# fudan-zvg/4d-gaussian-splatting

Measured on AMD Instinct MI355X. Metric: train-step images/sec + forward Mpix/s, 300k 4D Gaussians @1352x1014, higher is better.
Workload: dtype f32; 1 GPU; [model stored in Morton order, as fdgs.harness.train keeps it] C3: 300000 4D Gaussians, 1352x1014, SH degree 3 + time degree 2 (M=48), rot_4d=True, 4 views/GPU/step, L1+SSIM loss (fused HIP), Adam, fused activations, explicit fwd/loss/bwd on two HIP streams; num_rendered=2059257, cameras=4 different rotated off-axis cameras per step (fdgs.synth.POSES rig0..rig3), tile_cull=True, visible=254370, global_batch=4, parallelism=frame-parallel dp1, mode=weak scaling, 4 views per GPU and step (the reference's DyNeRF batch per GPU)

## Files before the change

4d-gaussian-splatting_amd/csrc/ssim.hip:

```cpp
#include <cstdlib>
#include "fdgs_common.h"

namespace fdgs
{
#ifndef FDGS_SSIM_STY
#define FDGS_SSIM_STY 32
#endif
	constexpr int STX = 32, STY = FDGS_SSIM_STY;
	constexpr int SROWS = STY / 8;
	constexpr int SR = 5;
	constexpr int SW = STX + 2 * SR;
	constexpr int SHH = STY + 2 * SR;
	constexpr int SSTR = 46;
	constexpr int SSTR1 = 48;
	constexpr int HSTR = 38;
	constexpr int HSTR1B = 36;
	constexpr int STHREADS = 256;
	typedef float v2f __attribute__((ext_vector_type(2)));
	typedef float v4f __attribute__((ext_vector_type(4)));

	struct TileId { int tx, ty, c, index; bool valid; };
	__device__ __forceinline__ TileId ssim_tile_of(int gx, int gy, int C)
	{
		const int total = gx * gy * C, chunk = (total + 7) / 8;
		const int wg = (int)blockIdx.x, xcd = wg & 7, k = wg >> 3;
		TileId t;
		t.index = xcd * chunk + k;
		t.valid = k < chunk && t.index < total;
		const int i = t.valid ? t.index : 0;
		t.c = i / (gx * gy);
		const int r = i - t.c * (gx * gy);
		t.ty = r / gx; t.tx = r - t.ty * gx;
		return t;
	}
	static inline int ssim_grid(int gx, int gy, int C) { return ((gx * gy * C + 7) / 8) * 8; }

	__device__ constexpr float GW[11] = {
		0.0010283801f, 0.0075987582f, 0.0360007733f, 0.1093606874f, 0.2130055279f, 0.2660117149f,
		0.2130055279f, 0.1093606874f, 0.0360007733f, 0.0075987582f, 0.0010283801f };

	__global__ void __launch_bounds__(STHREADS) ssim_fwd_kernel(
		const float* __restrict__ img1, const float* __restrict__ img2, int C, int H, int W,
		float* __restrict__ dm_dmu1, float* __restrict__ dm_de11, float* __restrict__ dm_de12,
		float* __restrict__ partial_l1, float* __restrict__ partial_ssim)
	{
		constexpr int IN_BYTES = SHH * SSTR * 8, HM_BYTES = SHH * HSTR * 8;
		constexpr int SH_BYTES = IN_BYTES > HM_BYTES ? IN_BYTES : HM_BYTES;
		__shared__ __attribute__((aligned(16))) char s_raw[HM_BYTES + SH_BYTES];
		v2f (*h_m)[HSTR] = reinterpret_cast<v2f (*)[HSTR]>(s_raw);
		v2f (*s_in)[SSTR] = reinterpret_cast<v2f (*)[SSTR]>(s_raw + HM_BYTES);
		v2f (*h_s)[HSTR] = reinterpret_cast<v2f (*)[HSTR]>(s_raw + HM_BYTES);
		__shared__ float red[2][STHREADS / WAVE];

		const TileId tile = ssim_tile_of((W + STX - 1) / STX, (H + STY - 1) / STY, C);
		if (!tile.valid) return;
		const int c = tile.c;
		const int x0 = tile.tx * STX, y0 = tile.ty * STY;
		const int tid = threadIdx.x;
		const size_t plane = (size_t)c * H * W;

		float l1 = 0.f;
		{
			constexpr int RPT = STHREADS / SW, TRIPS = (SHH + RPT - 1) / RPT;
			const int lyb = tid / SW, hx = tid - lyb * SW;
			const int gxh = x0 + hx - SR;
			const bool col_in = tid < RPT * SW && (unsigned)gxh < (unsigned)W;
			const bool col_own = (unsigned)(hx - SR) < (unsigned)STX;
			v2f p[TRIPS];
#pragma unroll
			for (int t = 0; t < TRIPS; t++)
			{
				const int ly = lyb + t * RPT, gy = y0 + ly - SR;
				const bool in = col_in && ly < SHH && (unsigned)gy < (unsigned)H;
				const size_t o = in ? plane + (size_t)gy * W + gxh : plane;
				const float vx = img1[o], vy = img2[o];
				p[t] = in ? v2f{ vx + vy, vx - vy } : v2f{ 0.0f, 0.0f };
			}
#pragma unroll
			for (int t = 0; t < TRIPS; t++)
			{
				const int ly = lyb + t * RPT;
				if (tid < RPT * SW && ly < SHH) s_in[ly][hx] = p[t];
				const bool own = col_own && (unsigned)(ly - SR) < (unsigned)STY;
				l1 += own ? fabsf(p[t].y) : 0.0f;
			}
		}
		__syncthreads();

		constexpr int HR = (SHH * (STX / 4) + STHREADS - 1) / STHREADS;
		v2f as[HR][4];
#pragma unroll
		for (int r = 0; r < HR; r++)
		{
			const int task = tid + r * STHREADS;
			if (task < SHH * (STX / 4))
			{
				const int ly = task >> 3, cx = (task & 7) * 4;
				v2f p[16], sq[14];
				const v4f* src = reinterpret_cast<const v4f*>(&s_in[ly][cx]);
#pragma unroll
				for (int i = 0; i < 7; i++) { const v4f q = src[i]; p[2 * i] = v2f{ q.x, q.y }; p[2 * i + 1] = v2f{ q.z, q.w }; }
#pragma unroll
				for (int i = 0; i < 14; i++) sq[i] = p[i] * p[i];
				v2f am[4];
#pragma unroll
				for (int j = 0; j < 4; j++)
				{
					am[j] = GW[0] * p[j]; as[r][j] = GW[0] * sq[j];
#pragma unroll
					for (int k = 1; k < 11; k++) { am[j] += GW[k] * p[j + k]; as[r][j] += GW[k] * sq[j + k]; }
				}
				v4f* dm = reinterpret_cast<v4f*>(&h_m[ly][cx]);
				dm[0] = v4f{ am[0].x, am[0].y, am[1].x, am[1].y }; dm[1] = v4f{ am[2].x, am[2].y, am[3].x, am[3].y };
			}
			__builtin_amdgcn_sched_barrier(0);
		}
		__syncthreads();
#pragma unroll
		for (int r = 0; r < HR; r++)
		{
			const int task = tid + r * STHREADS;
			if (task < SHH * (STX / 4))
			{
				const int ly = task >> 3, cx = (task & 7) * 4;
				v4f* ds = reinterpret_cast<v4f*>(&h_s[ly][cx]);
				ds[0] = v4f{ as[r][0].x, as[r][0].y, as[r][1].x, as[r][1].y }; ds[1] = v4f{ as[r][2].x, as[r][2].y, as[r][3].x, as[r][3].y };
			}
		}
		__syncthreads();

		const int lx = tid & (STX - 1), ly0 = (tid >> 5) * SROWS;
		v2f vm[10 + SROWS], vs[10 + SROWS];
#pragma unroll
		for (int r = 0; r < 10 + SROWS; r++) { vm[r] = h_m[ly0 + r][lx]; vs[r] = h_s[ly0 + r][lx]; }
		float sv = 0.f;
		const int gx = x0 + lx;
#pragma unroll
		for (int j = 0; j < SROWS; j++)
		{
			v2f mu = GW[0] * vm[j], e2 = GW[0] * vs[j];
#pragma unroll
			for (int k = 1; k < 11; k++) { mu += GW[k] * vm[j + k]; e2 += GW[k] * vs[j + k]; }
			const int gy = y0 + ly0 + j;
			if (gx < W && gy < H)
			{
				const float mu1 = 0.5f * (mu.x + mu.y), mu2 = 0.5f * (mu.x - mu.y);
				const float e_sum = 0.5f * (e2.x + e2.y), e12 = 0.25f * (e2.x - e2.y);
				const float C1 = 0.01f * 0.01f, C2 = 0.03f * 0.03f;
				const float mu1_sq = mu1 * mu1, mu2_sq = mu2 * mu2, mu12 = mu1 * mu2;
				const float sg12 = e12 - mu12;
				const float A = 2.f * mu12 + C1, B = 2.f * sg12 + C2, Cc = mu1_sq + mu2_sq + C1, D = (e_sum - (mu1_sq + mu2_sq)) + C2;
				const float rC = __builtin_amdgcn_rcpf(Cc), rD = __builtin_amdgcn_rcpf(D);
				const float inv = rC * rD;
				const float m = A * B * inv;
				const float dm_dA = B * inv, dm_dB = A * inv, dm_dC = -m * rC, dm_dD = -m * rD;
				const size_t o = plane + (size_t)gy * W + gx;
				dm_dmu1[o] = dm_dA * 2.f * mu2 - dm_dB * 2.f * mu2 + dm_dC * 2.f * mu1 - dm_dD * 2.f * mu1;
				dm_de11[o] = dm_dD;
				dm_de12[o] = 2.f * dm_dB;
				sv += m;
			}
		}
#pragma unroll
		for (int o = 32; o > 0; o >>= 1) { l1 += __shfl_down(l1, o); sv += __shfl_down(sv, o); }
		if ((tid & 63) == 0) { red[0][tid >> 6] = l1; red[1][tid >> 6] = sv; }
		__syncthreads();
		if (tid == 0)
		{
			const int b = tile.index;
			partial_l1[b] = red[0][0] + red[0][1] + red[0][2] + red[0][3];
			partial_ssim[b] = red[1][0] + red[1][1] + red[1][2] + red[1][3];
		}
	}

	__global__ void __launch_bounds__(STHREADS) ssim_bwd_kernel(
		const float* __restrict__ img1, const float* __restrict__ img2, int C, int H, int W,
		const float* __restrict__ dm_dmu1, const float* __restrict__ dm_de11, const float* __restrict__ dm_de12,
		const float* __restrict__ upstream, float w_l1, float w_ssim, float* __restrict__ dL_dimg1)
	{
		constexpr int SP_BYTES = SHH * SSTR * 8, SQ_BYTES = SHH * SSTR1 * 4, HP_BYTES = SHH * HSTR * 8, HQ_BYTES = SHH * HSTR1B * 4;
		constexpr int LDS_BYTES = SP_BYTES + SQ_BYTES > HP_BYTES + HQ_BYTES ? SP_BYTES + SQ_BYTES : HP_BYTES + HQ_BYTES;
		__shared__ __attribute__((aligned(16))) char s_raw[LDS_BYTES];
		v2f (*s_p)[SSTR] = reinterpret_cast<v2f (*)[SSTR]>(s_raw);
		float (*s_q)[SSTR1] = reinterpret_cast<float (*)[SSTR1]>(s_raw + SP_BYTES);
		v2f (*h_p)[HSTR] = reinterpret_cast<v2f (*)[HSTR]>(s_raw);
		float (*h_q)[HSTR1B] = reinterpret_cast<float (*)[HSTR1B]>(s_raw + HP_BYTES);

		const TileId tile = ssim_tile_of((W + STX - 1) / STX, (H + STY - 1) / STY, C);
		if (!tile.valid) return;
		const int c = tile.c;
		const int x0 = tile.tx * STX, y0 = tile.ty * STY;
		const int tid = threadIdx.x;
		const size_t plane = (size_t)c * H * W;

		{
			constexpr int RPT = STHREADS / SW, TRIPS = (SHH + RPT - 1) / RPT;
			const int lyb = tid / SW, hx = tid - lyb * SW;
			const int gxh = x0 + hx - SR;
			const bool col_in = tid < RPT * SW && (unsigned)gxh < (unsigned)W;
			v2f p[TRIPS];
			float q[TRIPS];
#pragma unroll
			for (int t = 0; t < TRIPS; t++)
			{
				const int ly = lyb + t * RPT, gy = y0 + ly - SR;
				const bool in = col_in && ly < SHH && (unsigned)gy < (unsigned)H;
				const size_t o = in ? plane + (size_t)gy * W + gxh : plane;
				const float va = dm_dmu1[o], vb = dm_de11[o], vc = dm_de12[o];
				p[t] = in ? v2f{ va, vb } : v2f{ 0.0f, 0.0f };
				q[t] = in ? vc : 0.0f;
			}
#pragma unroll
			for (int t = 0; t < TRIPS; t++)
			{
				const int ly = lyb + t * RPT;
				if (tid < RPT * SW && ly < SHH) { s_p[ly][hx] = p[t]; s_q[ly][hx] = q[t]; }
			}
		}
		const int lx = tid & (STX - 1), ly0 = (tid >> 5) * SROWS;
		const int gx = x0 + lx;
		float px[SROWS], py[SROWS];
#pragma unroll
		for (int j = 0; j < SROWS; j++)
		{
			const int gy = y0 + ly0 + j;
			const size_t o = (gx < W && gy < H) ? plane + (size_t)gy * W + gx : plane;
			px[j] = img1[o]; py[j] = img2[o];
		}
		__syncthreads();
		constexpr int HR = (SHH * (STX / 4) + STHREADS - 1) / STHREADS;
		v2f ap[HR][4];
		float aq[HR][4];
#pragma unroll
		for (int r = 0; r < HR; r++)
		{
			const int task = tid + r * STHREADS;
			if (task < SHH * (STX / 4))
			{
				const int ly = task >> 3, cx = (task & 7) * 4;
				v2f p[16];
				float q[16];
				const v4f* sp = reinterpret_cast<const v4f*>(&s_p[ly][cx]);
				const v4f* sq = reinterpret_cast<const v4f*>(&s_q[ly][cx]);
#pragma unroll
				for (int i = 0; i < 7; i++) { const v4f t = sp[i]; p[2 * i] = v2f{ t.x, t.y }; p[2 * i + 1] = v2f{ t.z, t.w }; }
#pragma unroll
				for (int i = 0; i < 4; i++) { const v4f t = sq[i]; q[4 * i] = t.x; q[4 * i + 1] = t.y; q[4 * i + 2] = t.z; q[4 * i + 3] = t.w; }
#pragma unroll
				for (int j = 0; j < 4; j++)
				{
					ap[r][j] = GW[0] * p[j]; aq[r][j] = GW[0] * q[j];
#pragma unroll
					for (int k = 1; k < 11; k++) { ap[r][j] += GW[k] * p[j + k]; aq[r][j] += GW[k] * q[j + k]; }
				}
			}
			__builtin_amdgcn_sched_barrier(0);
		}
		__syncthreads();
#pragma unroll
		for (int r = 0; r < HR; r++)
		{
			const int task = tid + r * STHREADS;
			if (task < SHH * (STX / 4))
			{
				const int ly = task >> 3, cx = (task & 7) * 4;
				v4f* dp = reinterpret_cast<v4f*>(&h_p[ly][cx]);
				dp[0] = v4f{ ap[r][0].x, ap[r][0].y, ap[r][1].x, ap[r][1].y }; dp[1] = v4f{ ap[r][2].x, ap[r][2].y, ap[r][3].x, ap[r][3].y };
				*reinterpret_cast<v4f*>(&h_q[ly][cx]) = v4f{ aq[r][0], aq[r][1], aq[r][2], aq[r][3] };
			}
		}
		__syncthreads();
		v2f vp[10 + SROWS];
		float vq[10 + SROWS];
#pragma unroll
		for (int r = 0; r < 10 + SROWS; r++) { vp[r] = h_p[ly0 + r][lx]; vq[r] = h_q[ly0 + r][lx]; }
		const float up = upstream[0];
#pragma unroll
		for (int j = 0; j < SROWS; j++)
		{
			v2f ab = GW[0] * vp[j];
			float d = GW[0] * vq[j];
#pragma unroll
			for (int k = 1; k < 11; k++) { ab += GW[k] * vp[j + k]; d += GW[k] * vq[j + k]; }
			const int gy = y0 + ly0 + j;
			if (gx < W && gy < H)
			{
				const size_t o = plane + (size_t)gy * W + gx;
				const float x = px[j], y = py[j];
				const float diff = x - y;
				const float sgn = diff > 0.f ? 1.f : (diff < 0.f ? -1.f : 0.f);
				dL_dimg1[o] = up * (w_l1 * sgn + w_ssim * (ab.x + 2.f * x * ab.y + y * d));
			}
		}
	}
}

namespace fdgs
{
	constexpr int FT = 32;
	constexpr int FB = FT + 2 * SR;
	constexpr int FA = FB + 2 * SR;
	constexpr int FBC = 44;
	constexpr int FSA = 54;
	constexpr int FSH = 46;
	constexpr int FSX = 48;
	constexpr int FSD = 46;
	constexpr int FSQ = 48;
	constexpr int FRV = 7;

	__device__ __forceinline__ void ssim_fused_body(
		const float* __restrict__ img1, const float* __restrict__ img2, int C, int H, int W,
		const float* __restrict__ upstream, float w_l1, float w_ssim, float* __restrict__ dL_dimg1,
		float* __restrict__ partial_l1, float* __restrict__ partial_ssim)
	{
		constexpr int R0_BYTES = FA * FSH * 8;
		constexpr int IN_BYTES = FA * FSA * 8, HS_BYTES = FA * FSH * 8, HX_BYTES = FA * FSX * 4;
		constexpr int R1_BYTES = IN_BYTES > HS_BYTES + HX_BYTES ? IN_BYTES : HS_BYTES + HX_BYTES;
		static_assert(FB * HSTR * 8 + FB * HSTR1B * 4 <= R0_BYTES, "h_p + h_q must fit where h_m was");
		static_assert(FB * FSD * 8 + FB * FSQ * 4 <= R1_BYTES, "d_p + d_q must fit where h_s + h_x were");
		__shared__ __attribute__((aligned(16))) char s_raw[R0_BYTES + R1_BYTES];
		v2f (*h_m)[FSH] = reinterpret_cast<v2f (*)[FSH]>(s_raw);
		v2f (*s_in)[FSA] = reinterpret_cast<v2f (*)[FSA]>(s_raw + R0_BYTES);
		v2f (*h_s)[FSH] = reinterpret_cast<v2f (*)[FSH]>(s_raw + R0_BYTES);
		float (*h_x)[FSX] = reinterpret_cast<float (*)[FSX]>(s_raw + R0_BYTES + HS_BYTES);
		v2f (*d_p)[FSD] = reinterpret_cast<v2f (*)[FSD]>(s_raw + R0_BYTES);
		float (*d_q)[FSQ] = reinterpret_cast<float (*)[FSQ]>(s_raw + R0_BYTES + FB * FSD * 8);
		v2f (*h_p)[HSTR] = reinterpret_cast<v2f (*)[HSTR]>(s_raw);
		float (*h_q)[HSTR1B] = reinterpret_cast<float (*)[HSTR1B]>(s_raw + FB * HSTR * 8);
		__shared__ float red[2][STHREADS / WAVE];

		const TileId tile = ssim_tile_of((W + FT - 1) / FT, (H + FT - 1) / FT, C);
		if (!tile.valid) return;
		const int c = tile.c;
		const int x0 = tile.tx * FT, y0 = tile.ty * FT;
		const int tid = threadIdx.x;
		const size_t plane = (size_t)c * H * W;

		float l1 = 0.f;
		{
			constexpr int RPT = STHREADS / FA, TRIPS = (FA + RPT - 1) / RPT;
			const int lyb = tid / FA, hx = tid - lyb * FA;
			const int gxh = x0 + hx - 2 * SR;
			const bool col_in = tid < RPT * FA && (unsigned)gxh < (unsigned)W;
			const bool col_own = (unsigned)(hx - 2 * SR) < (unsigned)FT;
			v2f p[TRIPS];
#pragma unroll
			for (int t = 0; t < TRIPS; t++)
			{
				const int ly = lyb + t * RPT, gy = y0 + ly - 2 * SR;
				const bool in = col_in && ly < FA && (unsigned)gy < (unsigned)H;
				const size_t o = in ? plane + (size_t)gy * W + gxh : plane;
				const float vx = img1[o], vy = img2[o];
				p[t] = in ? v2f{ vx, vy } : v2f{ 0.0f, 0.0f };
			}
#pragma unroll
			for (int t = 0; t < TRIPS; t++)
			{
				const int ly = lyb + t * RPT;
				if (tid < RPT * FA && ly < FA) s_in[ly][hx] = p[t];
				const bool own = col_own && (unsigned)(ly - 2 * SR) < (unsigned)FT;
				l1 += own ? fabsf(p[t].x - p[t].y) : 0.0f;
			}
			if (tid < FA) { s_in[tid][FA] = v2f{ 0.0f, 0.0f }; s_in[tid][FA + 1] = v2f{ 0.0f, 0.0f }; }
		}
		const int lx = tid & (FT - 1), ly0 = (tid >> 5) * SROWS;
		const int gx = x0 + lx;
		float px[SROWS], py[SROWS];
#pragma unroll
		for (int j = 0; j < SROWS; j++)
		{
			const int gy = y0 + ly0 + j;
			const size_t o = (gx < W && gy < H) ? plane + (size_t)gy * W + gx : plane;
			px[j] = img1[o]; py[j] = img2[o];
		}
		__syncthreads();

		{
			constexpr int GPR = FBC / 4, NT = FA * GPR, HR = (NT + STHREADS - 1) / STHREADS;
			v2f as[HR][4];
			float ax[HR][4];
#pragma unroll
			for (int r = 0; r < HR; r++)
			{
				const int task = tid + r * STHREADS;
				if (task < NT)
				{
					const int ly = task / GPR, cx = (task - ly * GPR) * 4;
					v2f p[16], sq[14];
					float xy[14];
					const v4f* src = reinterpret_cast<const v4f*>(&s_in[ly][cx]);
#pragma unroll
					for (int i = 0; i < 7; i++) { const v4f q = src[i]; p[2 * i] = v2f{ q.x, q.y }; p[2 * i + 1] = v2f{ q.z, q.w }; }
#pragma unroll
					for (int i = 0; i < 14; i++) { sq[i] = p[i] * p[i]; xy[i] = p[i].x * p[i].y; }
					v2f am[4];
#pragma unroll
					for (int j = 0; j < 4; j++)
					{
						am[j] = GW[0] * p[j]; as[r][j] = GW[0] * sq[j]; ax[r][j] = GW[0] * xy[j];
#pragma unroll
						for (int k = 1; k < 11; k++) { am[j] += GW[k] * p[j + k]; as[r][j] += GW[k] * sq[j + k]; ax[r][j] += GW[k] * xy[j + k]; }
					}
					v4f* dm = reinterpret_cast<v4f*>(&h_m[ly][cx]);
					dm[0] = v4f{ am[0].x, am[0].y, am[1].x, am[1].y }; dm[1] = v4f{ am[2].x, am[2].y, am[3].x, am[3].y };
				}
				__builtin_amdgcn_sched_barrier(0);
			}
			__syncthreads();
#pragma unroll
			for (int r = 0; r < HR; r++)
			{
				const int task = tid + r * STHREADS;
				if (task < NT)
				{
					const int ly = task / GPR, cx = (task - ly * GPR) * 4;
					v4f* ds = reinterpret_cast<v4f*>(&h_s[ly][cx]);
					ds[0] = v4f{ as[r][0].x, as[r][0].y, as[r][1].x, as[r][1].y }; ds[1] = v4f{ as[r][2].x, as[r][2].y, as[r][3].x, as[r][3].y };
					*reinterpret_cast<v4f*>(&h_x[ly][cx]) = v4f{ ax[r][0], ax[r][1], ax[r][2], ax[r][3] };
				}
			}
		}
		__syncthreads();

		float sv = 0.f;
		{
			const int bc = tid % FB, rg = tid / FB;
			const bool work = rg < FB / FRV;
			const int br0 = work ? rg * FRV : 0;
			v2f dp[FRV];
			float dq[FRV];
			{
				v2f vm[10 + FRV], vs[10 + FRV];
				float vx[10 + FRV];
#pragma unroll
				for (int r = 0; r < 10 + FRV; r++) { vm[r] = h_m[br0 + r][bc]; vs[r] = h_s[br0 + r][bc]; vx[r] = h_x[br0 + r][bc]; }
				const int gxb = x0 + bc - SR;
				const bool col_own = (unsigned)(bc - SR) < (unsigned)FT;
#pragma unroll
				for (int j = 0; j < FRV; j++)
				{
					v2f mu = GW[0] * vm[j], e2 = GW[0] * vs[j];
					float e12 = GW[0] * vx[j];
#pragma unroll
					for (int k = 1; k < 11; k++) { mu += GW[k] * vm[j + k]; e2 += GW[k] * vs[j + k]; e12 += GW[k] * vx[j + k]; }
					const int br = br0 + j, gyb = y0 + br - SR;
					dp[j] = v2f{ 0.0f, 0.0f }; dq[j] = 0.0f;
					if (work && (unsigned)gxb < (unsigned)W && (unsigned)gyb < (unsigned)H)
					{
						const float mu1 = mu.x, mu2 = mu.y, e11 = e2.x, e22 = e2.y;
						const float C1 = 0.01f * 0.01f, C2 = 0.03f * 0.03f;
						const float mu1_sq = mu1 * mu1, mu2_sq = mu2 * mu2, mu12 = mu1 * mu2;
						const float sg1 = e11 - mu1_sq, sg2 = e22 - mu2_sq, sg12 = e12 - mu12;
						const float A = 2.f * mu12 + C1, B = 2.f * sg12 + C2, Cc = mu1_sq + mu2_sq + C1, D = sg1 + sg2 + C2;
						const float rC = __builtin_amdgcn_rcpf(Cc), rD = __builtin_amdgcn_rcpf(D);
						const float inv = rC * rD;
						const float m = A * B * inv;
						const float dm_dA = B * inv, dm_dB = A * inv, dm_dC = -m * rC, dm_dD = -m * rD;
						dp[j] = v2f{ dm_dA * 2.f * mu2 - dm_dB * 2.f * mu2 + dm_dC * 2.f * mu1 - dm_dD * 2.f * mu1, dm_dD };
						dq[j] = 2.f * dm_dB;
						if (col_own && (unsigned)(br - SR) < (unsigned)FT) sv += m;
					}
				}
			}
			__syncthreads();
			if (work)
			{
#pragma unroll
				for (int j = 0; j < FRV; j++) { d_p[br0 + j][bc] = dp[j]; d_q[br0 + j][bc] = dq[j]; }
			}
			if (tid < FB) { d_q[tid][FB] = 0.0f; d_q[tid][FB + 1] = 0.0f; d_q[tid][FB + 2] = 0.0f; d_q[tid][FB + 3] = 0.0f; }
		}
		__syncthreads();

		{
			constexpr int NT = FB * (FT / 4), HR = (NT + STHREADS - 1) / STHREADS;
#pragma unroll
			for (int r = 0; r < HR; r++)
			{
				const int task = tid + r * STHREADS;
				if (task < NT)
				{
					const int ly = task >> 3, cx = (task & 7) * 4;
					v2f p[16];
					float q[16];
					const v4f* sp = reinterpret_cast<const v4f*>(&d_p[ly][cx]);
					const v4f* sq = reinterpret_cast<const v4f*>(&d_q[ly][cx]);
#pragma unroll
					for (int i = 0; i < 7; i++) { const v4f t = sp[i]; p[2 * i] = v2f{ t.x, t.y }; p[2 * i + 1] = v2f{ t.z, t.w }; }
#pragma unroll
					for (int i = 0; i < 4; i++) { const v4f t = sq[i]; q[4 * i] = t.x; q[4 * i + 1] = t.y; q[4 * i + 2] = t.z; q[4 * i + 3] = t.w; }
					v2f ap[4];
					float aq[4];
#pragma unroll
					for (int j = 0; j < 4; j++)
					{
						ap[j] = GW[0] * p[j]; aq[j] = GW[0] * q[j];
#pragma unroll
						for (int k = 1; k < 11; k++) { ap[j] += GW[k] * p[j + k]; aq[j] += GW[k] * q[j + k]; }
					}
					v4f* dpo = reinterpret_cast<v4f*>(&h_p[ly][cx]);
					dpo[0] = v4f{ ap[0].x, ap[0].y, ap[1].x, ap[1].y }; dpo[1] = v4f{ ap[2].x, ap[2].y, ap[3].x, ap[3].y };
					*reinterpret_cast<v4f*>(&h_q[ly][cx]) = v4f{ aq[0], aq[1], aq[2], aq[3] };
				}
				__builtin_amdgcn_sched_barrier(0);
			}
		}
		__syncthreads();

		{
			v2f vp[10 + SROWS];
			float vq[10 + SROWS];
#pragma unroll
			for (int r = 0; r < 10 + SROWS; r++) { vp[r] = h_p[ly0 + r][lx]; vq[r] = h_q[ly0 + r][lx]; }
			const float up = upstream[0];
#pragma unroll
			for (int j = 0; j < SROWS; j++)
			{
				v2f ab = GW[0] * vp[j];
				float d = GW[0] * vq[j];
#pragma unroll
				for (int k = 1; k < 11; k++) { ab += GW[k] * vp[j + k]; d += GW[k] * vq[j + k]; }
				const int gy = y0 + ly0 + j;
				if (gx < W && gy < H)
				{
					const size_t o = plane + (size_t)gy * W + gx;
					const float x = px[j], y = py[j];
					const float diff = x - y;
					const float sgn = diff > 0.f ? 1.f : (diff < 0.f ? -1.f : 0.f);
					dL_dimg1[o] = up * (w_l1 * sgn + w_ssim * (ab.x + 2.f * x * ab.y + y * d));
				}
			}
		}
#pragma unroll
		for (int o = 32; o > 0; o >>= 1) { l1 += __shfl_down(l1, o); sv += __shfl_down(sv, o); }
		if ((tid & 63) == 0) { red[0][tid >> 6] = l1; red[1][tid >> 6] = sv; }
		__syncthreads();
		if (tid == 0)
		{
			const int b = tile.index;
			partial_l1[b] = red[0][0] + red[0][1] + red[0][2] + red[0][3];
			partial_ssim[b] = red[1][0] + red[1][1] + red[1][2] + red[1][3];
		}
	}
}

namespace fdgs
{
#define FDGS_SSIM_FUSED_PARAMS const float* __restrict__ img1, const float* __restrict__ img2, int C, int H, int W, const float* __restrict__ upstream, \
		float w_l1, float w_ssim, float* __restrict__ dL_dimg1, float* __restrict__ partial_l1, float* __restrict__ partial_ssim
	__global__ void __launch_bounds__(STHREADS) __attribute__((amdgpu_waves_per_eu(3, 3))) ssim_fused_kernel(FDGS_SSIM_FUSED_PARAMS)
	{
		ssim_fused_body(img1, img2, C, H, W, upstream, w_l1, w_ssim, dL_dimg1, partial_l1, partial_ssim);
	}
	__global__ void __launch_bounds__(STHREADS) ssim_fused_kernel_wpe2(FDGS_SSIM_FUSED_PARAMS)
	{
		ssim_fused_body(img1, img2, C, H, W, upstream, w_l1, w_ssim, dL_dimg1, partial_l1, partial_ssim);
	}
#undef FDGS_SSIM_FUSED_PARAMS
}

extern "C" int fdgs_l1_ssim_value_and_grad(const float* img, const float* gt, int32_t C, int32_t H, int32_t W,
                                           const float* upstream, float lambda_dssim, float* dL_dimg,
                                           float* partial_l1, float* partial_ssim, void* stream)
{
	using namespace fdgs;
	static_assert(STY == 32 && SROWS == 4, "the fused kernel shares the 32-row tile's partial-sum layout with the two-kernel path");
	if (!img || !gt || !upstream || !dL_dimg || !partial_l1 || !partial_ssim || C <= 0 || H <= 0 || W <= 0) return FDGS_ERR_INVALID_ARG;
	const float n = (float)C * (float)H * (float)W;
	const float w_l1 = (1.0f - lambda_dssim) / n, w_ssim = -lambda_dssim / n;
	const dim3 grid(ssim_grid(div_up(W, FT), div_up(H, FT), C)), block(STHREADS, 1, 1);
	static const bool wpe2 = []() { const char* e = getenv("FDGS_SSIM_FUSED_WPE"); return e && e[0] == '2'; }();
	if (wpe2) hipLaunchKernelGGL(ssim_fused_kernel_wpe2, grid, block, 0, (hipStream_t)stream, img, gt, C, H, W, upstream, w_l1, w_ssim, dL_dimg, partial_l1, partial_ssim);
	else hipLaunchKernelGGL(ssim_fused_kernel, grid, block, 0, (hipStream_t)stream, img, gt, C, H, W, upstream, w_l1, w_ssim, dL_dimg, partial_l1, partial_ssim);
	return hipGetLastError() == hipSuccess ? FDGS_OK : FDGS_ERR_HIP;
}

extern "C" int fdgs_l1_ssim_forward(const float* img, const float* gt, int32_t C, int32_t H, int32_t W,
                                    float* dm_dmu1, float* dm_de11, float* dm_de12,
                                    float* partial_l1, float* partial_ssim, void* stream)
{
	using namespace fdgs;
	if (!img || !gt || !dm_dmu1 || !dm_de11 || !dm_de12 || !partial_l1 || !partial_ssim || C <= 0 || H <= 0 || W <= 0) return FDGS_ERR_INVALID_ARG;
	const dim3 grid(ssim_grid(div_up(W, STX), div_up(H, STY), C)), block(STHREADS, 1, 1);
	hipLaunchKernelGGL(ssim_fwd_kernel, grid, block, 0, (hipStream_t)stream, img, gt, C, H, W, dm_dmu1, dm_de11, dm_de12, partial_l1, partial_ssim);
	return hipGetLastError() == hipSuccess ? FDGS_OK : FDGS_ERR_HIP;
}

extern "C" int fdgs_l1_ssim_backward(const float* img, const float* gt, int32_t C, int32_t H, int32_t W,
                                     const float* dm_dmu1, const float* dm_de11, const float* dm_de12,
                                     const float* upstream, float lambda_dssim, float* dL_dimg, void* stream)
{
	using namespace fdgs;
	if (!img || !gt || !dm_dmu1 || !dm_de11 || !dm_de12 || !upstream || !dL_dimg || C <= 0 || H <= 0 || W <= 0) return FDGS_ERR_INVALID_ARG;
	const float n = (float)C * (float)H * (float)W;
	const float w_l1 = (1.0f - lambda_dssim) / n, w_ssim = -lambda_dssim / n;
	const dim3 grid(ssim_grid(div_up(W, STX), div_up(H, STY), C)), block(STHREADS, 1, 1);
	hipLaunchKernelGGL(ssim_bwd_kernel, grid, block, 0, (hipStream_t)stream, img, gt, C, H, W, dm_dmu1, dm_de11, dm_de12, upstream, w_l1, w_ssim, dL_dimg);
	return hipGetLastError() == hipSuccess ? FDGS_OK : FDGS_ERR_HIP;
}

namespace fdgs
{
	__global__ void __launch_bounds__(1024) l1_ssim_finish_kernel(const float* __restrict__ partial_l1, const float* __restrict__ partial_ssim,
	                                                              int nparts, float inv_n, float lambda_dssim, float* __restrict__ out, long long view_stride)
	{
		partial_l1 += (size_t)blockIdx.x * view_stride; partial_ssim += (size_t)blockIdx.x * view_stride; out += 3 * (size_t)blockIdx.x;
		__shared__ float r0[16], r1[16];
		float a = 0.f, b = 0.f;
		for (int base = 0; base < nparts; base += 8 * 1024)
		{
			float va[8], vb[8];
#pragma unroll
			for (int k = 0; k < 8; k++)
			{
				const int i = base + k * 1024 + (int)threadIdx.x;
				va[k] = i < nparts ? partial_l1[i] : 0.f;
				vb[k] = i < nparts ? partial_ssim[i] : 0.f;
			}
			a += ((va[0] + va[1]) + (va[2] + va[3])) + ((va[4] + va[5]) + (va[6] + va[7]));
			b += ((vb[0] + vb[1]) + (vb[2] + vb[3])) + ((vb[4] + vb[5]) + (vb[6] + vb[7]));
		}
#pragma unroll
		for (int o = 32; o > 0; o >>= 1) { a += __shfl_xor(a, o); b += __shfl_xor(b, o); }
		if ((threadIdx.x & 63) == 0) { r0[threadIdx.x >> 6] = a; r1[threadIdx.x >> 6] = b; }
		__syncthreads();
		if (threadIdx.x == 0)
		{
			float s0 = 0.f, s1 = 0.f;
			for (int w = 0; w < 16; w++) { s0 += r0[w]; s1 += r1[w]; }
			const float l1 = s0 * inv_n, ss = s1 * inv_n;
			out[0] = (1.0f - lambda_dssim) * l1 + lambda_dssim * (1.0f - ss);
			out[1] = l1;
			out[2] = ss;
		}
	}
}

extern "C" int fdgs_l1_ssim_loss(const float* partial_l1, const float* partial_ssim, int32_t num_partials, int32_t C, int32_t H, int32_t W,
                                 float lambda_dssim, float* loss_l1_ssim, void* stream)
{
	using namespace fdgs;
	if (!partial_l1 || !partial_ssim || !loss_l1_ssim || num_partials <= 0 || C <= 0 || H <= 0 || W <= 0) return FDGS_ERR_INVALID_ARG;
	const float inv_n = 1.0f / ((float)C * (float)H * (float)W);
	hipLaunchKernelGGL(l1_ssim_finish_kernel, dim3(1), dim3(1024), 0, (hipStream_t)stream, partial_l1, partial_ssim, num_partials, inv_n, lambda_dssim, loss_l1_ssim, 0ll);
	return hipGetLastError() == hipSuccess ? FDGS_OK : FDGS_ERR_HIP;
}

extern "C" int fdgs_l1_ssim_loss_batch(const float* partials, int32_t num_views, int32_t num_partials, int32_t C, int32_t H, int32_t W,
                                       float lambda_dssim, float* losses, void* stream)
{
	using namespace fdgs;
	if (!partials || !losses || num_views <= 0 || num_partials <= 0 || C <= 0 || H <= 0 || W <= 0) return FDGS_ERR_INVALID_ARG;
	const float inv_n = 1.0f / ((float)C * (float)H * (float)W);
	hipLaunchKernelGGL(l1_ssim_finish_kernel, dim3(num_views), dim3(1024), 0, (hipStream_t)stream, partials, partials + num_partials, num_partials, inv_n,
	                   lambda_dssim, losses, 2ll * num_partials);
	return hipGetLastError() == hipSuccess ? FDGS_OK : FDGS_ERR_HIP;
}

extern "C" int fdgs_l1_ssim_num_partials(int32_t C, int32_t H, int32_t W)
{
	using namespace fdgs;
	return div_up(W, STX) * div_up(H, STY) * C;
}
```

Measured before the change: 2435 images/s.

## Reorder SSIM separable blur to vertical-in-registers then horizontal-from-LDS with vector stores

Rewrites the standalone SSIM forward and backward kernels. Each thread now loads a 6-row column strip from global memory straight into registers and does the vertical 11-tap blur there, with a fast unguarded path for interior tiles. The horizontal blur then runs from a single LDS buffer, with each thread producing 4 adjacent pixels and writing them with 16-byte vector stores when rows are aligned. This removes the raw-input LDS staging, one intermediate LDS pass and two barriers, in exchange for more registers per thread and some overlap between row groups, which recompute a few rows.

```diff
diff --git a/4d-gaussian-splatting_amd/csrc/ssim.hip b/4d-gaussian-splatting_amd/csrc/ssim.hip
--- a/4d-gaussian-splatting_amd/csrc/ssim.hip
+++ b/4d-gaussian-splatting_amd/csrc/ssim.hip
@@ -39,17 +39,37 @@
 		0.0010283801f, 0.0075987582f, 0.0360007733f, 0.1093606874f, 0.2130055279f, 0.2660117149f,
 		0.2130055279f, 0.1093606874f, 0.0360007733f, 0.0075987582f, 0.0010283801f };
 
+	constexpr int VR = 6;
+	constexpr int VG = (STY + VR - 1) / VR;
+	constexpr int VIN = VR + 2 * SR;
+	constexpr int VSTR4 = 43;
+	static_assert(STY == 32 && STX == 32 && VG * SW <= STHREADS && STY * (STX / 4) == STHREADS, "thread maps of the two passes");
+
+	__device__ __forceinline__ bool halo_inside(int x0, int y0, int H, int W)
+	{
+		return x0 >= SR && x0 + STX + SR <= W && y0 >= SR && y0 + STY + SR <= H && W < (1 << 24);
+	}
+	__device__ __forceinline__ bool rows_aligned16(int W, const void* a, const void* b, const void* c, const void* d = nullptr)
+	{
+		return (W & 3) == 0 && (((uintptr_t)a | (uintptr_t)b | (uintptr_t)c | (uintptr_t)d) & 15) == 0;
+	}
+	__device__ __forceinline__ void store4(float* __restrict__ dst, size_t o, const float (&v)[4], bool vec, int nvalid)
+	{
+		if (nvalid <= 0) return;
+		if (vec) *reinterpret_cast<v4f*>(dst + o) = v4f{ v[0], v[1], v[2], v[3] };
+		else
+		{
+#pragma unroll
+			for (int j = 0; j < 4; j++) if (j < nvalid) dst[o + j] = v[j];
+		}
+	}
+
 	__global__ void __launch_bounds__(STHREADS) ssim_fwd_kernel(
 		const float* __restrict__ img1, const float* __restrict__ img2, int C, int H, int W,
 		float* __restrict__ dm_dmu1, float* __restrict__ dm_de11, float* __restrict__ dm_de12,
 		float* __restrict__ partial_l1, float* __restrict__ partial_ssim)
 	{
-		constexpr int IN_BYTES = SHH * SSTR * 8, HM_BYTES = SHH * HSTR * 8;
-		constexpr int SH_BYTES = IN_BYTES > HM_BYTES ? IN_BYTES : HM_BYTES;
-		__shared__ __attribute__((aligned(16))) char s_raw[HM_BYTES + SH_BYTES];
-		v2f (*h_m)[HSTR] = reinterpret_cast<v2f (*)[HSTR]>(s_raw);
-		v2f (*s_in)[SSTR] = reinterpret_cast<v2f (*)[SSTR]>(s_raw + HM_BYTES);
-		v2f (*h_s)[HSTR] = reinterpret_cast<v2f (*)[HSTR]>(s_raw + HM_BYTES);
+		__shared__ __attribute__((aligned(16))) v4f s_v[STY][VSTR4];
 		__shared__ float red[2][STHREADS / WAVE];
 
 		const TileId tile = ssim_tile_of((W + STX - 1) / STX, (H + STY - 1) / STY, C);
@@ -60,90 +80,72 @@
 		const size_t plane = (size_t)c * H * W;
 
 		float l1 = 0.f;
-		{
-			constexpr int RPT = STHREADS / SW, TRIPS = (SHH + RPT - 1) / RPT;
-			const int lyb = tid / SW, hx = tid - lyb * SW;
+		if (tid < VG * SW)
+		{
+			const int g = tid / SW, hx = tid - g * SW;
+			const int r0 = g * VR < STY - VR ? g * VR : STY - VR;
 			const int gxh = x0 + hx - SR;
-			const bool col_in = tid < RPT * SW && (unsigned)gxh < (unsigned)W;
+			const bool col_in = (unsigned)gxh < (unsigned)W;
 			const bool col_own = (unsigned)(hx - SR) < (unsigned)STX;
-			v2f p[TRIPS];
-#pragma unroll
-			for (int t = 0; t < TRIPS; t++)
-			{
-				const int ly = lyb + t * RPT, gy = y0 + ly - SR;
-				const bool in = col_in && ly < SHH && (unsigned)gy < (unsigned)H;
-				const size_t o = in ? plane + (size_t)gy * W + gxh : plane;
-				const float vx = img1[o], vy = img2[o];
-				p[t] = in ? v2f{ vx + vy, vx - vy } : v2f{ 0.0f, 0.0f };
-			}
-#pragma unroll
-			for (int t = 0; t < TRIPS; t++)
-			{
-				const int ly = lyb + t * RPT;
-				if (tid < RPT * SW && ly < SHH) s_in[ly][hx] = p[t];
-				const bool own = col_own && (unsigned)(ly - SR) < (unsigned)STY;
-				l1 += own ? fabsf(p[t].y) : 0.0f;
-			}
-		}
-		__syncthreads();
-
-		constexpr int HR = (SHH * (STX / 4) + STHREADS - 1) / STHREADS;
-		v2f as[HR][4];
-#pragma unroll
-		for (int r = 0; r < HR; r++)
-		{
-			const int task = tid + r * STHREADS;
-			if (task < SHH * (STX / 4))
-			{
-				const int ly = task >> 3, cx = (task & 7) * 4;
-				v2f p[16], sq[14];
-				const v4f* src = reinterpret_cast<const v4f*>(&s_in[ly][cx]);
-#pragma unroll
-				for (int i = 0; i < 7; i++) { const v4f q = src[i]; p[2 * i] = v2f{ q.x, q.y }; p[2 * i + 1] = v2f{ q.z, q.w }; }
-#pragma unroll
-				for (int i = 0; i < 14; i++) sq[i] = p[i] * p[i];
-				v2f am[4];
-#pragma unroll
-				for (int j = 0; j < 4; j++)
-				{
-					am[j] = GW[0] * p[j]; as[r][j] = GW[0] * sq[j];
-#pragma unroll
-					for (int k = 1; k < 11; k++) { am[j] += GW[k] * p[j + k]; as[r][j] += GW[k] * sq[j + k]; }
-				}
-				v4f* dm = reinterpret_cast<v4f*>(&h_m[ly][cx]);
-				dm[0] = v4f{ am[0].x, am[0].y, am[1].x, am[1].y }; dm[1] = v4f{ am[2].x, am[2].y, am[3].x, am[3].y };
-			}
-			__builtin_amdgcn_sched_barrier(0);
-		}
-		__syncthreads();
-#pragma unroll
-		for (int r = 0; r < HR; r++)
-		{
-			const int task = tid + r * STHREADS;
-			if (task < SHH * (STX / 4))
-			{
-				const int ly = task >> 3, cx = (task & 7) * 4;
-				v4f* ds = reinterpret_cast<v4f*>(&h_s[ly][cx]);
-				ds[0] = v4f{ as[r][0].x, as[r][0].y, as[r][1].x, as[r][1].y }; ds[1] = v4f{ as[r][2].x, as[r][2].y, as[r][3].x, as[r][3].y };
-			}
-		}
-		__syncthreads();
-
-		const int lx = tid & (STX - 1), ly0 = (tid >> 5) * SROWS;
-		v2f vm[10 + SROWS], vs[10 + SROWS];
-#pragma unroll
-		for (int r = 0; r < 10 + SROWS; r++) { vm[r] = h_m[ly0 + r][lx]; vs[r] = h_s[ly0 + r][lx]; }
+			const float* __restrict__ c1 = img1 + plane + (col_in ? gxh : 0);
+			const float* __restrict__ c2 = img2 + plane + (col_in ? gxh : 0);
+			v2f p[VIN], sq[VIN];
+			float vx[VIN], vy[VIN];
+			if (halo_inside(x0, y0, H, W))
+			{
+				const unsigned voff = (unsigned)(r0 * W + gxh) * 4u;
+#pragma unroll
+				for (int i = 0; i < VIN; i++)
+				{
+					const size_t row = plane + (size_t)(y0 - SR + i) * W;
+					vx[i] = *reinterpret_cast<const float*>(reinterpret_cast<const char*>(img1 + row) + voff);
+					vy[i] = *reinterpret_cast<const float*>(reinterpret_cast<const char*>(img2 + row) + voff);
+				}
+			}
+			else
+			{
+#pragma unroll
+				for (int i = 0; i < VIN; i++)
+				{
+					const int gy = y0 + r0 + i - SR;
+					const bool in = col_in && (unsigned)gy < (unsigned)H;
+					const size_t o = in ? (size_t)gy * W : 0;
+					const float a = c1[o], b = c2[o];
+					vx[i] = in ? a : 0.0f; vy[i] = in ? b : 0.0f;
+				}
+			}
+#pragma unroll
+			for (int i = 0; i < VIN; i++) p[i] = v2f{ vx[i] + vy[i], vx[i] - vy[i] };
+#pragma unroll
+			for (int i = 0; i < VIN; i++) sq[i] = p[i] * p[i];
+#pragma unroll
+			for (int j = 0; j < VR; j++)
+			{
+				v2f m = GW[0] * p[j], s = GW[0] * sq[j];
+#pragma unroll
+				for (int k = 1; k < 11; k++) { m += GW[k] * p[j + k]; s += GW[k] * sq[j + k]; }
+				s_v[r0 + j][hx] = v4f{ m.x, m.y, s.x, s.y };
+				const bool own = col_own && r0 + j >= g * VR;
+				l1 += own ? fabsf(p[j + SR].y) : 0.0f;
+			}
+		}
+		__syncthreads();
+
+		const int ly = tid >> 3, cx = (tid & 7) * 4;
+		const int gy = y0 + ly, gx0 = x0 + cx;
 		float sv = 0.f;
-		const int gx = x0 + lx;
-#pragma unroll
-		for (int j = 0; j < SROWS; j++)
-		{
-			v2f mu = GW[0] * vm[j], e2 = GW[0] * vs[j];
-#pragma unroll
-			for (int k = 1; k < 11; k++) { mu += GW[k] * vm[j + k]; e2 += GW[k] * vs[j + k]; }
-			const int gy = y0 + ly0 + j;
-			if (gx < W && gy < H)
-			{
+		float o_mu1[4], o_e11[4], o_e12[4];
+		{
+			v4f q[14];
+			const v4f* src = &s_v[ly][cx];
+#pragma unroll
+			for (int i = 0; i < 14; i++) q[i] = src[i];
+#pragma unroll
+			for (int j = 0; j < 4; j++)
+			{
+				v2f mu = GW[0] * q[j].xy, e2 = GW[0] * q[j].zw;
+#pragma unroll
+				for (int k = 1; k < 11; k++) { mu += GW[k] * q[j + k].xy; e2 += GW[k] * q[j + k].zw; }
 				const float mu1 = 0.5f * (mu.x + mu.y), mu2 = 0.5f * (mu.x - mu.y);
 				const float e_sum = 0.5f * (e2.x + e2.y), e12 = 0.25f * (e2.x - e2.y);
 				const float C1 = 0.01f * 0.01f, C2 = 0.03f * 0.03f;
@@ -154,12 +156,19 @@
 				const float inv = rC * rD;
 				const float m = A * B * inv;
 				const float dm_dA = B * inv, dm_dB = A * inv, dm_dC = -m * rC, dm_dD = -m * rD;
-				const size_t o = plane + (size_t)gy * W + gx;
-				dm_dmu1[o] = dm_dA * 2.f * mu2 - dm_dB * 2.f * mu2 + dm_dC * 2.f * mu1 - dm_dD * 2.f * mu1;
-				dm_de11[o] = dm_dD;
-				dm_de12[o] = 2.f * dm_dB;
-				sv += m;
-			}
+				o_mu1[j] = dm_dA * 2.f * mu2 - dm_dB * 2.f * mu2 + dm_dC * 2.f * mu1 - dm_dD * 2.f * mu1;
+				o_e11[j] = dm_dD;
+				o_e12[j] = 2.f * dm_dB;
+				sv += (gx0 + j < W && gy < H) ? m : 0.0f;
+			}
+		}
+		{
+			const bool vec = rows_aligned16(W, dm_dmu1, dm_de11, dm_de12);
+			const int nvalid = gy < H ? W - gx0 : 0;
+			const size_t o = plane + (size_t)(gy < H ? gy : 0) * W + gx0;
+			store4(dm_dmu1, o, o_mu1, vec, nvalid);
+			store4(dm_de11, o, o_e11, vec, nvalid);
+			store4(dm_de12, o, o_e12, vec, nvalid);
 		}
 #pragma unroll
 		for (int o = 32; o > 0; o >>= 1) { l1 += __shfl_down(l1, o); sv += __shfl_down(sv, o); }
@@ -178,13 +187,8 @@
 		const float* __restrict__ dm_dmu1, const float* __restrict__ dm_de11, const float* __restrict__ dm_de12,
 		const float* __restrict__ upstream, float w_l1, float w_ssim, float* __restrict__ dL_dimg1)
 	{
-		constexpr int SP_BYTES = SHH * SSTR * 8, SQ_BYTES = SHH * SSTR1 * 4, HP_BYTES = SHH * HSTR * 8, HQ_BYTES = SHH * HSTR1B * 4;
-		constexpr int LDS_BYTES = SP_BYTES + SQ_BYTES > HP_BYTES + HQ_BYTES ? SP_BYTES + SQ_BYTES : HP_BYTES + HQ_BYTES;
-		__shared__ __attribute__((aligned(16))) char s_raw[LDS_BYTES];
-		v2f (*s_p)[SSTR] = reinterpret_cast<v2f (*)[SSTR]>(s_raw);
-		float (*s_q)[SSTR1] = reinterpret_cast<float (*)[SSTR1]>(s_raw + SP_BYTES);
-		v2f (*h_p)[HSTR] = reinterpret_cast<v2f (*)[HSTR]>(s_raw);
-		float (*h_q)[HSTR1B] = reinterpret_cast<float (*)[HSTR1B]>(s_raw + HP_BYTES);
+		__shared__ __attribute__((aligned(16))) v2f s_p[STY][SSTR];
+		__shared__ __attribute__((aligned(16))) float s_q[STY][SSTR1];
 
 		const TileId tile = ssim_tile_of((W + STX - 1) / STX, (H + STY - 1) / STY, C);
 		if (!tile.valid) return;
@@ -193,105 +197,94 @@
 		const int tid = threadIdx.x;
 		const size_t plane = (size_t)c * H * W;
 
-		{
-			constexpr int RPT = STHREADS / SW, TRIPS = (SHH + RPT - 1) / RPT;
-			const int lyb = tid / SW, hx = tid - lyb * SW;
+		if (tid < VG * SW)
+		{
+			const int g = tid / SW, hx = tid - g * SW;
+			const int r0 = g * VR < STY - VR ? g * VR : STY - VR;
 			const int gxh = x0 + hx - SR;
-			const bool col_in = tid < RPT * SW && (unsigned)gxh < (unsigned)W;
-			v2f p[TRIPS];
-			float q[TRIPS];
-#pragma unroll
-			for (int t = 0; t < TRIPS; t++)
-			{
-				const int ly = lyb + t * RPT, gy = y0 + ly - SR;
-				const bool in = col_in && ly < SHH && (unsigned)gy < (unsigned)H;
-				const size_t o = in ? plane + (size_t)gy * W + gxh : plane;
-				const float va = dm_dmu1[o], vb = dm_de11[o], vc = dm_de12[o];
-				p[t] = in ? v2f{ va, vb } : v2f{ 0.0f, 0.0f };
-				q[t] = in ? vc : 0.0f;
-			}
-#pragma unroll
-			for (int t = 0; t < TRIPS; t++)
-			{
-				const int ly = lyb + t * RPT;
-				if (tid < RPT * SW && ly < SHH) { s_p[ly][hx] = p[t]; s_q[ly][hx] = q[t]; }
-			}
-		}
-		const int lx = tid & (STX - 1), ly0 = (tid >> 5) * SROWS;
-		const int gx = x0 + lx;
-		float px[SROWS], py[SROWS];
-#pragma unroll
-		for (int j = 0; j < SROWS; j++)
-		{
-			const int gy = y0 + ly0 + j;
-			const size_t o = (gx < W && gy < H) ? plane + (size_t)gy * W + gx : plane;
-			px[j] = img1[o]; py[j] = img2[o];
-		}
-		__syncthreads();
-		constexpr int HR = (SHH * (STX / 4) + STHREADS - 1) / STHREADS;
-		v2f ap[HR][4];
-		float aq[HR][4];
-#pragma unroll
-		for (int r = 0; r < HR; r++)
-		{
-			const int task = tid + r * STHREADS;
-			if (task < SHH * (STX / 4))
-			{
-				const int ly = task >> 3, cx = (task & 7) * 4;
-				v2f p[16];
-				float q[16];
-				const v4f* sp = reinterpret_cast<const v4f*>(&s_p[ly][cx]);
-				const v4f* sq = reinterpret_cast<const v4f*>(&s_q[ly][cx]);
-#pragma unroll
-				for (int i = 0; i < 7; i++) { const v4f t = sp[i]; p[2 * i] = v2f{ t.x, t.y }; p[2 * i + 1] = v2f{ t.z, t.w }; }
-#pragma unroll
-				for (int i = 0; i < 4; i++) { const v4f t = sq[i]; q[4 * i] = t.x; q[4 * i + 1] = t.y; q[4 * i + 2] = t.z; q[4 * i + 3] = t.w; }
-#pragma unroll
-				for (int j = 0; j < 4; j++)
-				{
-					ap[r][j] = GW[0] * p[j]; aq[r][j] = GW[0] * q[j];
-#pragma unroll
-					for (int k = 1; k < 11; k++) { ap[r][j] += GW[k] * p[j + k]; aq[r][j] += GW[k] * q[j + k]; }
-				}
-			}
-			__builtin_amdgcn_sched_barrier(0);
-		}
-		__syncthreads();
-#pragma unroll
-		for (int r = 0; r < HR; r++)
-		{
-			const int task = tid + r * STHREADS;
-			if (task < SHH * (STX / 4))
-			{
-				const int ly = task >> 3, cx = (task & 7) * 4;
-				v4f* dp = reinterpret_cast<v4f*>(&h_p[ly][cx]);
-				dp[0] = v4f{ ap[r][0].x, ap[r][0].y, ap[r][1].x, ap[r][1].y }; dp[1] = v4f{ ap[r][2].x, ap[r][2].y, ap[r][3].x, ap[r][3].y };
-				*reinterpret_cast<v4f*>(&h_q[ly][cx]) = v4f{ aq[r][0], aq[r][1], aq[r][2], aq[r][3] };
-			}
-		}
-		__syncthreads();
-		v2f vp[10 + SROWS];
-		float vq[10 + SROWS];
-#pragma unroll
-		for (int r = 0; r < 10 + SROWS; r++) { vp[r] = h_p[ly0 + r][lx]; vq[r] = h_q[ly0 + r][lx]; }
+			const bool col_in = (unsigned)gxh < (unsigned)W;
+			const size_t cb = plane + (col_in ? gxh : 0);
+			v2f p[VIN];
+			float q[VIN];
+			if (halo_inside(x0, y0, H, W))
+			{
+				const unsigned voff = (unsigned)(r0 * W + gxh) * 4u;
+#pragma unroll
+				for (int i = 0; i < VIN; i++)
+				{
+					const size_t row = plane + (size_t)(y0 - SR + i) * W;
+					p[i].x = *reinterpret_cast<const float*>(reinterpret_cast<const char*>(dm_dmu1 + row) + voff);
+					p[i].y = *reinterpret_cast<const float*>(reinterpret_cast<const char*>(dm_de11 + row) + voff);
+					q[i] = *reinterpret_cast<const float*>(reinterpret_cast<const char*>(dm_de12 + row) + voff);
+				}
+			}
+			else
+			{
+#pragma unroll
+				for (int i = 0; i < VIN; i++)
+				{
+					const int gy = y0 + r0 + i - SR;
+					const bool in = col_in && (unsigned)gy < (unsigned)H;
+					const size_t o = cb + (in ? (size_t)gy * W : 0);
+					const float va = dm_dmu1[o], vb = dm_de11[o], vc = dm_de12[o];
+					p[i] = in ? v2f{ va, vb } : v2f{ 0.0f, 0.0f };
+					q[i] = in ? vc : 0.0f;
+				}
+			}
+#pragma unroll
+			for (int j = 0; j < VR; j++)
+			{
+				v2f ab = GW[0] * p[j];
+				float d = GW[0] * q[j];
+#pragma unroll
+				for (int k = 1; k < 11; k++) { ab += GW[k] * p[j + k]; d += GW[k] * q[j + k]; }
+				s_p[r0 + j][hx] = ab; s_q[r0 + j][hx] = d;
+			}
+		}
+		const int ly = tid >> 3, cx = (tid & 7) * 4;
+		const int gy = y0 + ly, gx0 = x0 + cx;
+		const bool vec = rows_aligned16(W, img1, img2, dL_dimg1);
+		const int nvalid = gy < H ? W - gx0 : 0;
+		const size_t o = plane + (size_t)(gy < H ? gy : 0) * W + gx0;
+		float px[4], py[4];
+		if (vec)
+		{
+			const size_t ov = nvalid > 0 ? o : plane;
+			const v4f a = *reinterpret_cast<const v4f*>(img1 + ov), b = *reinterpret_cast<const v4f*>(img2 + ov);
+			px[0] = a.x; px[1] = a.y; px[2] = a.z; px[3] = a.w; py[0] = b.x; py[1] = b.y; py[2] = b.z; py[3] = b.w;
+		}
+		else
+		{
+#pragma unroll
+			for (int j = 0; j < 4; j++) { const size_t oj = j < nvalid ? o + j : plane; px[j] = img1[oj]; py[j] = img2[oj]; }
+		}
 		const float up = upstream[0];
-#pragma unroll
-		for (int j = 0; j < SROWS; j++)
-		{
-			v2f ab = GW[0] * vp[j];
-			float d = GW[0] * vq[j];
-#pragma unroll
-			for (int k = 1; k < 11; k++) { ab += GW[k] * vp[j + k]; d += GW[k] * vq[j + k]; }
-			const int gy = y0 + ly0 + j;
-			if (gx < W && gy < H)
-			{
-				const size_t o = plane + (size_t)gy * W + gx;
+		__syncthreads();
+
+		float out[4];
+		{
+			v2f p[16];
+			float q[16];
+			const v4f* sp = reinterpret_cast<const v4f*>(&s_p[ly][cx]);
+			const v4f* sq = reinterpret_cast<const v4f*>(&s_q[ly][cx]);
+#pragma unroll
+			for (int i = 0; i < 7; i++) { const v4f t = sp[i]; p[2 * i] = t.xy; p[2 * i + 1] = t.zw; }
+#pragma unroll
+			for (int i = 0; i < 4; i++) { const v4f t = sq[i]; q[4 * i] = t.x; q[4 * i + 1] = t.y; q[4 * i + 2] = t.z; q[4 * i + 3] = t.w; }
+#pragma unroll
+			for (int j = 0; j < 4; j++)
+			{
+				v2f ab = GW[0] * p[j];
+				float d = GW[0] * q[j];
+#pragma unroll
+				for (int k = 1; k < 11; k++) { ab += GW[k] * p[j + k]; d += GW[k] * q[j + k]; }
 				const float x = px[j], y = py[j];
 				const float diff = x - y;
 				const float sgn = diff > 0.f ? 1.f : (diff < 0.f ? -1.f : 0.f);
-				dL_dimg1[o] = up * (w_l1 * sgn + w_ssim * (ab.x + 2.f * x * ab.y + y * d));
-			}
-		}
+				out[j] = up * (w_l1 * sgn + w_ssim * (ab.x + 2.f * x * ab.y + y * d));
+			}
+		}
+		store4(dL_dimg1, o, out, vec, nvalid);
 	}
 }
 
```

Result: slower. 2368 images/s (-2.7%).
